# AlvinYH/Faster-VoxelPose

Hardware: AMD Instinct MI355X
Metric: frames/sec at 5-view 80x80x20 voxel (heatmaps -> 3D joints); MPJPE vs ref (mm) in mpjpe_vs_ref_mm (higher is better)
Workload: dtype f32

## Files before the change

faster-voxelpose_amd/csrc/fvp_project.hip:

```cpp
#include <hip/hip_runtime.h>

#include <cfloat>
#include <climits>
#include <cstdlib>

#include "fvp_common.h"
#include "fvp_geom.h"

namespace fvp {

template <int NV>
__global__ void __launch_bounds__(256) k_heat_to_cl(const float* __restrict__ heat, float* __restrict__ cl,
                                                    int J, int HW) {
  const int pix = blockIdx.x * 256 + threadIdx.x;
  const size_t bv = blockIdx.y;
  if (pix >= HW) return;
  const float* src = heat + bv * size_t(J) * HW + pix;
  float v[4 * NV];
#pragma unroll
  for (int j = 0; j < 4 * NV; ++j) v[j] = (j < J) ? src[size_t(j) * HW] : 0.0f;
  float4* dst = reinterpret_cast<float4*>(cl + (bv * HW + pix) * size_t(4 * NV));
#pragma unroll
  for (int q = 0; q < NV; ++q) dst[q] = make_float4(v[4 * q], v[4 * q + 1], v[4 * q + 2], v[4 * q + 3]);
}
// ... 1360 lines not shown
  if (B == 0) return 0;
  ProfScope ps(FVP_K_PROJECT_WHOLE, as_stream(s));
  const int threads = ceil_div(4 * Z, 64) * 64;
  if (g->JP <= 16)
    hipLaunchKernelGGL(k_project_columns_q<1>, dim3(B * N), dim3(threads), 0, as_stream(s), heat_cl,
                       reinterpret_cast<const Cam*>(cams), frame_set, ax, ay, az, Y, Z, X * Y, N, *g,
                       reinterpret_cast<const long long*>(flat), feat1d);
  else
    hipLaunchKernelGGL(k_project_columns_q<2>, dim3(B * N), dim3(threads), 0, as_stream(s), heat_cl,
                       reinterpret_cast<const Cam*>(cams), frame_set, ax, ay, az, Y, Z, X * Y, N, *g,
                       reinterpret_cast<const long long*>(flat), feat1d);
  return launch_status();
}

extern "C" int fvp_zmax(const float* cubes, float* zmax, long n, int Z, fvp_stream_t s) {
  FVP_REQUIRE(cubes && zmax && n >= 0 && Z > 0);
  if (n == 0) return 0;
  hipLaunchKernelGGL(k_zmax, dim3(unsigned((n + 255) / 256)), dim3(256), 0, as_stream(s), cubes, zmax, n, Z);
  return launch_status();
}

extern "C" int fvp_person_boxes(const float* centers, int n, const float* consts, const int32_t* fine_cube,
                                int32_t* boxes, float* offset, fvp_stream_t s) {
  FVP_REQUIRE(centers && consts && fine_cube && boxes && offset && n >= 0);
  if (n == 0) return 0;
  hipLaunchKernelGGL(k_person_boxes, dim3(ceil_div(n, 64)), dim3(64), 0, as_stream(s), centers, n, consts,
                     fine_cube[0], fine_cube[1], fine_cube[2], fine_cube[3], fine_cube[4], fine_cube[5], boxes,
                     offset);
  return launch_status();
}

extern "C" int fvp_plane_live_rows(const int32_t* boxes, int nP, int C, int32_t* live_rows, fvp_stream_t s) {
  FVP_REQUIRE(boxes && live_rows && nP >= 0 && C > 0);
  if (nP == 0) return 0;
  hipLaunchKernelGGL(k_plane_live_rows, dim3(ceil_div(nP, 64)), dim3(64), 0, as_stream(s), boxes, nP, C, live_rows);
  return launch_status();
}

static int check_cube(int C) {
  if (C < 4 || C > 256 || (C & (C - 1)) != 0) return FVP_ELIMIT;
  return 0;
}

extern "C" int fvp_project_individual(const float* heat_cl, const float* cams, const int32_t* frame_set,
                                      const int32_t* person_frame, const uint8_t* person_valid,
                                      const int32_t* boxes, const float* fx, const float* fy, const float* fz,
                                      const int32_t* fine, int C, int nP, const FvpGeom* g, float* cubes,
                                      fvp_stream_t s) {
  FVP_REQUIRE(heat_cl && cams && frame_set && person_frame && boxes && fx && fy && fz && cubes && nP >= 0);
  (void)fine;
  if (int e = check_geom(g)) return e;
  if (int e = check_cube(C)) return e;
  if (nP == 0) return 0;
  ProfScope ps(FVP_K_OTHER, as_stream(s));
#define CALL(NV)                                                                                                 \
  auto k = &k_project_individual<NV>;                                                                            \
  hipLaunchKernelGGL(k, dim3(ceil_div(C * C * C, 256), nP), dim3(256), 0, as_stream(s), heat_cl,                 \
                     reinterpret_cast<const Cam*>(cams), frame_set, person_frame, person_valid, boxes, fx, fy, fz, \
                     C, *g, cubes);
  FVP_NV_SWITCH(g->JP / 4, CALL)
#undef CALL
  return launch_status();
}

extern "C" int fvp_triplane_max(const float* cubes, float* planes, int nP, int J, int C, fvp_stream_t s) {
  FVP_REQUIRE(cubes && planes && nP >= 0 && J > 0);
  if (int e = check_cube(C)) return e;
  FVP_LIMIT(C <= 128);
  if (nP == 0) return 0;
  ProfScope ps(FVP_K_OTHER, as_stream(s));
  const int per = (C * C + 255) / 256;
  const dim3 grid(J, nP);
  const size_t lds = size_t(C) * (C + 1) * sizeof(float);
#define FVP_TRIMAX(PER_) hipLaunchKernelGGL(k_triplane_max<PER_>, grid, dim3(256), lds, as_stream(s), cubes, planes, J, C)
  if (per <= 1) FVP_TRIMAX(1);
  else if (per <= 4) FVP_TRIMAX(4);
  else if (per <= 16) FVP_TRIMAX(16);
  else FVP_TRIMAX(64);
#undef FVP_TRIMAX
  return launch_status();
}

static int tri_owned_ny(int C) { return ceil_div(C, kBY); }

extern "C" int fvp_project_individual_triplane(const float* heat_cl, const float* cams, const int32_t* frame_set,
                                               const int32_t* person_frame, const uint8_t* person_valid,
                                               const int32_t* boxes, const float* fx, const float* fy,
                                               const float* fz, const int32_t* fine, int C, int nP, const FvpGeom* g,
                                               float* planes, int persons_per_frame, const float* fine_grid,
                                               fvp_stream_t s) {
  FVP_REQUIRE(heat_cl && cams && frame_set && person_frame && boxes && fx && fy && fz && planes && nP >= 0);
  FVP_REQUIRE(!fine_grid || fine);
  if (int e = check_geom(g)) return e;
  if (int e = check_cube(C)) return e;
  if (nP == 0) return 0;
  const int ppf = (persons_per_frame > 0 && nP % persons_per_frame == 0) ? persons_per_frame : nP;
  [[maybe_unused]] const int chunks = ceil_div(C * C, 256);
  const int nvl = ceil_div(g->JP, 16);
  ProfScope ps(FVP_K_PROJECT_TRIPLANE, as_stream(s));
  const int F0 = fine_grid ? fine[0] : 0, F1 = fine_grid ? fine[1] : 0, F2 = fine_grid ? fine[2] : 0;
  const int nby = ceil_div(C, kBY);
#if FVP_DIAG
  const int nbx = ceil_div(C, kBX);
  static const bool gather = fvp::diag_env("FVP_TRIPLANE_GATHER") != nullptr;
  const bool quad_form = fvp::diag_env("FVP_TRIPLANE_QUAD") != nullptr;
  static const int tri_ablate_env = fvp::diag_env("FVP_TRI_ABLATE") ? atoi(fvp::diag_env("FVP_TRI_ABLATE")) : 0;
  const char* tt_env = fvp::diag_env("FVP_TRI_TWO_TILE");
  const bool staged = fvp::diag_env("FVP_TRIPLANE_STAGED") != nullptr;
  const bool force_lane = fvp::diag_env("FVP_TRIPLANE_LANE") != nullptr;
  const bool lane_form = !gather && !quad_form && g->JP <= 20 && ((staged && g->JP != 16) || force_lane);
  const int tri_ablate = (tri_ablate_env & ~16) | ((tt_env ? atoi(tt_env) != 0 : lane_form) ? 16 : 0);
  auto cap_lim = [](int cap) { const char* e = fvp::diag_env("FVP_TRI_CAP_PX"); const int v = e ? atoi(e) : cap; return v > 0 && v < cap ? v : cap; };
  const int cap_px = int((36 * 1024) / (size_t(g->JP) * 4));
  const size_t lds = 2 * size_t(cap_px) * g->JP * 4 + 64;
  if (lane_form) {
    const int lq = (g->JP / 4) | 1;
    const int cap_px = int((36 * 1024) / (size_t(lq) * 16));
    const size_t lds = 2 * size_t(cap_px) * lq * 16 + 64;
    FVP_LIMIT(size_t(cap_px) * lq * 4 >= size_t(kBX * kBY + (kBX + kBY) * 32) * g->JP);
#define CALL2(NQ_, CACHED_)                                                                                       \
  {                                                                                                                \
    static LdsOptIn optin;                                                                                         \
    auto k = &k_project_triplane_lds2<NQ_, CACHED_>;                                                              \
    if (int e = lds_opt_in(optin, reinterpret_cast<const void*>(k), lds)) return e;                                \
    hipLaunchKernelGGL(k, dim3(nbx * nby * nP), dim3(kTriThreads), lds, as_stream(s), heat_cl,                     \
                       reinterpret_cast<const Cam*>(cams), frame_set, person_frame, person_valid, boxes, fx, fy, fz, C, \
                       nP, nbx, nby, ppf, cap_px, *g, fine_grid, F0, F1, F2, planes, tri_ablate, cap_lim(cap_px));                  \
  }
#define CASE2(NQ_) case NQ_: if (fine_grid) CALL2(NQ_, true) else CALL2(NQ_, false) break;
    switch (g->JP / 4) {
      CASE2(1) CASE2(2) CASE2(3) CASE2(4) CASE2(5)
      default: return FVP_ELIMIT;
    }
#undef CASE2
#undef CALL2
    return launch_status();
  }
  const bool blk_form = !gather && !quad_form && !staged;
#else
  constexpr bool blk_form = true;
#endif
  if (blk_form && nvl <= 2) {
    const int nbx2 = ceil_div(C, kBlkBX);
    const int bz = nvl == 2 ? 16 : kBlkBZ;
    int zsh = 0;
    while ((1 << zsh) < C) ++zsh;
    const size_t lds_z = (size_t(kBlkBX + kBY) << zsh) * (g->JP + 1) * 4;
#if FVP_DIAG
    const char* zr_env = fvp::diag_env("FVP_TRI_ZRES");
    const bool zres = zr_env && atoi(zr_env) != 0 && (1 << zsh) >= bz && lds_z <= kTriZresMaxLds;
#else
    constexpr bool zres = false;
#endif
    const bool fits32 = (long long)g->H * g->W * g->JP * g->V <= INT_MAX && (long long)F0 * F1 * F2 * g->V <= INT_MAX;
    bool owned = tri_owned_lds(C, g->JP) <= kTriOwnMaxLds && fits32 && !zres;
    int ny = tri_owned_ny(C);
#if FVP_DIAG
    if (const char* e = fvp::diag_env("FVP_TRI_OWNED")) owned = owned && atoi(e) != 0;
    if (const char* e = fvp::diag_env("FVP_TRI_NY")) {
      const int v = atoi(e), top = ceil_div(C, kBY);
      ny = v < 1 ? 1 : (v > top ? top : v);
    }
#endif
    if (owned) {
      const int nsx = ceil_div(C, kOwnSX);
      int zsh_o = 0;
      while ((1 << zsh_o) < C || (1 << zsh_o) < kOwnBZ) ++zsh_o;
      const size_t lds_o = tri_owned_lds(C, g->JP);
      const bool q5o = nvl == 2 && g->JP == 20 && fvp::diag_env("FVP_TRI_NO_Q5") == nullptr;
#define CALLO(NVL_, CACHED_, Q5_)                                                                                            \
  hipLaunchKernelGGL((k_project_triplane_own<NVL_, CACHED_, Q5_>), dim3(nsx * ny * nP), dim3(kOwnThreads), lds_o,           \
                     as_stream(s), heat_cl, reinterpret_cast<const Cam*>(cams), frame_set, person_frame, person_valid, boxes, \
                     fx, fy, fz, C, nP, nsx, ny, ppf, *g, fine_grid, F0, F1, F2, planes, zsh_o)
      if (q5o) { if (fine_grid) CALLO(2, true, true); else CALLO(2, false, true); }
      else if (nvl == 2) { if (fine_grid) CALLO(2, true, false); else CALLO(2, false, false); }
      else { if (fine_grid) CALLO(1, true, false); else CALLO(1, false, false); }
#undef CALLO
      return launch_status();
    }
    const size_t lds_b = zres ? lds_z : size_t(kBlkBX * kBY + (kBlkBX + kBY) * bz) * (g->JP + 1) * 4;
#define CALLB(NVL_, CACHED_, ZRES_)                                                                                          \
  hipLaunchKernelGGL((k_project_triplane_blk<NVL_, CACHED_, ZRES_>), dim3(nbx2 * nby * nP), dim3(kBlkThreads), lds_b,       \
                     as_stream(s), heat_cl, reinterpret_cast<const Cam*>(cams), frame_set, person_frame, person_valid, boxes, \
                     fx, fy, fz, C, nP, nbx2, nby, ppf, *g, fine_grid, F0, F1, F2, planes, zsh)
#if FVP_DIAG
#define CALLB2(NVL_)                                                                     \
  {                                                                                      \
    if (fine_grid) { if (zres) CALLB(NVL_, true, true); else CALLB(NVL_, true, false); } \
    else { if (zres) CALLB(NVL_, false, true); else CALLB(NVL_, false, false); }         \
  }
#else
#define CALLB2(NVL_)                                                                     \
  {                                                                                      \
    if (fine_grid) CALLB(NVL_, true, false); else CALLB(NVL_, false, false);             \
  }
#endif
    const bool q5 = nvl == 2 && g->JP == 20 && !zres && fvp::diag_env("FVP_TRI_NO_Q5") == nullptr;
    if (q5) {
      if (fine_grid)
        hipLaunchKernelGGL((k_project_triplane_blk<2, true, false, true>), dim3(nbx2 * nby * nP), dim3(kBlkThreads), lds_b, as_stream(s),
                           heat_cl, reinterpret_cast<const Cam*>(cams), frame_set, person_frame, person_valid, boxes, fx, fy, fz, C, nP,
                           nbx2, nby, ppf, *g, fine_grid, F0, F1, F2, planes, zsh);
      else
        hipLaunchKernelGGL((k_project_triplane_blk<2, false, false, true>), dim3(nbx2 * nby * nP), dim3(kBlkThreads), lds_b, as_stream(s),
                           heat_cl, reinterpret_cast<const Cam*>(cams), frame_set, person_frame, person_valid, boxes, fx, fy, fz, C, nP,
                           nbx2, nby, ppf, *g, fine_grid, F0, F1, F2, planes, zsh);
    } else if (nvl == 2) CALLB2(2) else CALLB2(1)
#undef CALLB2
#undef CALLB
    return launch_status();
  }
#if FVP_DIAG
  if (!gather && nvl <= 2) {
    FVP_LIMIT(cap_px >= kBX * kBY + (kBX + kBY) * (nvl == 1 ? 32 : 16));
#define CALL(NVL_, CACHED_)                                                                                        \
  {                                                                                                                \
    static LdsOptIn optin;                                                                                         \
    auto k = &k_project_triplane_lds<NVL_, CACHED_>;                                                               \
    if (int e = lds_opt_in(optin, reinterpret_cast<const void*>(k), lds)) return e;                                \
    hipLaunchKernelGGL(k, dim3(nbx * nby * nP), dim3(kTriThreads), lds, as_stream(s), heat_cl,                     \
                       reinterpret_cast<const Cam*>(cams), frame_set, person_frame, person_valid, boxes, fx, fy, fz, C, \
                       nP, nbx, nby, ppf, cap_px, *g, fine_grid, F0, F1, F2, planes, tri_ablate, cap_lim(cap_px));                  \
  }
    if (nvl == 1) {
      if (fine_grid) CALL(1, true) else CALL(1, false)
    } else {
      if (fine_grid) CALL(2, true) else CALL(2, false)
    }
#undef CALL
    return launch_status();
  }
  if (nvl == 1) {
    auto k = &k_project_triplane<1>;
    hipLaunchKernelGGL(k, dim3(chunks * nP), dim3(1024), 0, as_stream(s), heat_cl, reinterpret_cast<const Cam*>(cams),
                       frame_set, person_frame, person_valid, boxes, fx, fy, fz, C, nP, chunks, ppf, *g, planes);
  } else if (nvl == 2) {
    auto k = &k_project_triplane<2>;
    hipLaunchKernelGGL(k, dim3(chunks * nP), dim3(1024), 0, as_stream(s), heat_cl, reinterpret_cast<const Cam*>(cams),
                       frame_set, person_frame, person_valid, boxes, fx, fy, fz, C, nP, chunks, ppf, *g, planes);
  } else {
    return FVP_ELIMIT;
  }
  return launch_status();
#else
  return FVP_ELIMIT;
#endif
}
```

faster-voxelpose_amd/csrc/fvp_project_lds.h:

```cpp
#pragma once
#include <type_traits>
#include <climits>

namespace fvp {

typedef float f32x2 __attribute__((ext_vector_type(2)));
#ifndef FVP_TRI_PACKED
#define FVP_TRI_PACKED 1
#endif
#ifndef FVP_TRI_EXPLICIT_AS
#define FVP_TRI_EXPLICIT_AS 1
#endif

typedef float f32x4v __attribute__((ext_vector_type(4)));
__device__ __forceinline__ float4 lds_ld4(const float* p) {
  const f32x4v v = *(const __attribute__((address_space(3))) f32x4v*)p;
  return make_float4(v.x, v.y, v.z, v.w);
}
__device__ __forceinline__ float4 glb_ld4(const float* p) {
  const f32x4v v = *(const __attribute__((address_space(1))) f32x4v*)p;
  return make_float4(v.x, v.y, v.z, v.w);
}

struct TapL {
// ... 552 lines not shown
    if (acc[0][0][0] != 1.2345e-30f) continue;
#endif
    if constexpr (ZRES) {
      int* rxz = reinterpret_cast<int*>(smem);
      int* ryz = rxz + ((kBX << zsh) * JPp);
      const int zb = gz0 - s2 + zs;
#pragma unroll
      for (int n = 0; n < NVL; ++n)
#pragma unroll
        for (int c = 0; c < 4; ++c) {
          const int ch = 16 * n + 4 * q + c;
          float mz = 0.0f;
#pragma unroll
          for (int i = 0; i < VPT; ++i) {
            const float val = fmaxf(acc[i][n][c], 0.0f);
            mz = fmaxf(mz, val);
            if (val > 0.0f && ch < JP) {
              const int z = zb + 4 * i;
              atomicMax(&rxz[((xx << zsh) + z) * JPp + ch], __float_as_int(val));
              atomicMax(&ryz[((yy << zsh) + z) * JPp + ch], __float_as_int(val));
            }
          }
          int mi = __float_as_int(mz);
          mi = imax(mi, dpp_i<0x124>(mi));
          mi = imax(mi, dpp_i<0x128>(mi));
          mxy[n][c] = imax(mxy[n][c], mi);
        }
      continue;
    }
    int* cxy = reinterpret_cast<int*>(smem);
    int* cxz = cxy + kBX * kBY * JPp;
    int* cyz = cxz + kBX * BZ * JPp;
    const int ncell = (kBX * kBY + (kBX + kBY) * BZ) * JPp;
    __syncthreads();
    for (int i = t; i < ncell; i += NT) cxy[i] = 0;
    __syncthreads();
#pragma unroll
    for (int n = 0; n < NVA; ++n)
#pragma unroll
      for (int c = 0; c < 4; ++c) {
        const int ch = 16 * n + 4 * q + c;
        float mz = 0.0f;
#pragma unroll
        for (int i = 0; i < VPT; ++i) {
          const float val = fmaxf(acc[i][n][c], 0.0f);
          mz = fmaxf(mz, val);
          if (val > 0.0f && ch < JP) {
            const int z = zs + 4 * i;
            atomicMax(&cxz[(xx * BZ + z) * JPp + ch], __float_as_int(val));
            atomicMax(&cyz[(yy * BZ + z) * JPp + ch], __float_as_int(val));
          }
        }
        int mi = __float_as_int(mz);
        mi = imax(mi, dpp_i<0x124>(mi));
        mi = imax(mi, dpp_i<0x128>(mi));
        if (zs == 0 && mi > 0 && ch < JP) cxy[(xx * kBY + yy) * JPp + ch] = mi;
      }
    if constexpr (Q5) {
#pragma unroll
      for (int c = 0; c < 4; ++c) {
        const int ch = 16 + c;
        float mz = 0.0f;
#pragma unroll
        for (int kk = 0; kk < OWN; ++kk) {
          const float val = fmaxf(accx[kk][0][c], 0.0f);
          mz = fmaxf(mz, val);
          if (val > 0.0f) {
            const int z = zs + 4 * (4 * kk + q);
            atomicMax(&cxz[(xx * BZ + z) * JPp + ch], __float_as_int(val));
            atomicMax(&cyz[(yy * BZ + z) * JPp + ch], __float_as_int(val));
          }
        }
        int mi = __float_as_int(mz);
        mi = imax(mi, dpp_i<0x121>(mi));
        mi = imax(mi, dpp_i<0x122>(mi));
        mi = imax(mi, dpp_i<0x124>(mi));
        mi = imax(mi, dpp_i<0x128>(mi));
        if (zs == 0 && q == 0 && mi > 0) cxy[(xx * kBY + yy) * JPp + ch] = mi;
      }
    }
    __syncthreads();
    const int lz0 = gz0 - tl2;
    for (int i = t; i < kBX * kBY * J; i += NT) {
      const int ch = i / (kBX * kBY), col = i - ch * (kBX * kBY), cx = col / kBY, cy = col - cx * kBY;
      const int raw = cxy[col * JPp + ch];
      if (raw > 0 && gx0 + cx < e0 && gy0 + cy < e1) {
        const int vv = __float_as_int(clampf(__fdiv_rn(__int_as_float(raw), nv), 0.0f, 1.0f));
        if (vv > 0) plane_max(&pxy[size_t(ch) * CC + (gx0 + cx - tl0) * C + (gy0 + cy - tl1)], vv);
      }
    }
    for (int i = t; i < (kBX + kBY) * BZ * J; i += NT) {
      const int ch = i / ((kBX + kBY) * BZ), r = i - ch * ((kBX + kBY) * BZ), a = r / BZ, z = r - a * BZ;
      if (gz0 + z < e2) {
        const int raw = cxz[r * JPp + ch];
        const int vv = raw > 0 ? __float_as_int(clampf(__fdiv_rn(__int_as_float(raw), nv), 0.0f, 1.0f)) : 0;
        if (vv > 0) {
          if (a < kBX) {
            if (gx0 + a < e0) plane_max(&pxz[size_t(ch) * CC + (gx0 + a - tl0) * C + lz0 + z], vv);
          } else if (gy0 + a - kBX < e1) {
            plane_max(&pyz[size_t(ch) * CC + (gy0 + a - kBX - tl1) * C + lz0 + z], vv);
          }
        }
      }
    }
  }
  if constexpr (ZRES) {
    __syncthreads();
    if (zs == 0 && col_in) {
#pragma unroll
      for (int n = 0; n < NVL; ++n)
#pragma unroll
        for (int c = 0; c < 4; ++c) {
          const int ch = 16 * n + 4 * q + c;
          if (ch < J && mxy[n][c] > 0) {
            const int vv = __float_as_int(clampf(__fdiv_rn(__int_as_float(mxy[n][c]), nv), 0.0f, 1.0f));
            if (vv > 0) plane_max(&pxy[size_t(ch) * CC + (gxi - tl0) * C + (gyi - tl1)], vv);
          }
        }
    }
    const int* cz = reinterpret_cast<const int*>(smem);
    const int nz = e2 - s2, lz0 = s2 - tl2;
    const int rows = (kBX + kBY) << zsh;
    for (int i = t; i < rows * J; i += NT) {
      static_assert(kBX + kBY == 8, "row count is a power of two");
      const int ch = i >> (zsh + 3), r = i & (rows - 1), a = r >> zsh, z = r & (zt - 1);
      if (z < nz) {
        const int raw = cz[r * JPp + ch];
        const int vv = raw > 0 ? __float_as_int(clampf(__fdiv_rn(__int_as_float(raw), nv), 0.0f, 1.0f)) : 0;
        if (vv > 0) {
          if (a < kBX) {
            if (gx0 + a < e0) plane_max(&pxz[size_t(ch) * CC + (gx0 + a - tl0) * C + lz0 + z], vv);
          } else if (gy0 + a - kBX < e1) {
            plane_max(&pyz[size_t(ch) * CC + (gy0 + a - kBX - tl1) * C + lz0 + z], vv);
          }
        }
      }
    }
  }
}

constexpr int kOwnSX = 4;
constexpr int kOwnBZ = 16;
constexpr int kOwnThreads = kOwnSX * kBY * 4 * 4;
#ifndef FVP_TRI_OWN_MAX_KB
#define FVP_TRI_OWN_MAX_KB 36
#endif
constexpr size_t kTriOwnMaxLds = size_t(FVP_TRI_OWN_MAX_KB) * 1024;
constexpr int kOwnPar = 16;
inline size_t tri_owned_lds(int C, int JP) {
  const int zt = C > kOwnBZ ? C : kOwnBZ;
  return (size_t(kOwnSX) * zt + 2 * size_t(kBY) * kOwnBZ) * size_t(JP + 1) * 4 + 4 * kOwnPar;
}

template <int NVL, bool CACHED, bool Q5 = false>
__global__ void __launch_bounds__(kOwnThreads, FVP_TRI_BLK_OCC)
k_project_triplane_own(const float* __restrict__ heat_cl, const Cam* __restrict__ cams, const int* __restrict__ frame_set,
                       const int* __restrict__ person_frame, const uint8_t* __restrict__ person_valid,
                       const int* __restrict__ boxes, const float* __restrict__ fx, const float* __restrict__ fy,
                       const float* __restrict__ fz, int C, int nP, int nsx, int ny, int ppf, FvpGeom g,
                       const float* __restrict__ fgrid, int F0, int F1, int F2, float* __restrict__ planes, int zsh) {
  static_assert(!Q5 || NVL == 2, "the five-quad form replaces the two-group form");
  constexpr int NVA = Q5 ? 1 : NVL;
  constexpr int BZ = kOwnBZ, VPT = BZ / 4, OWN = VPT / 4, SX = kOwnSX, NT = kOwnThreads;
  HIP_DYNAMIC_SHARED(float, smem)
  const int J = g.J, JP = g.JP, V = g.V, W = g.W, H = g.H;
  int p, blk;
  {
    const int id = blockIdx.x;
    const int bpp = nsx * ny, bpf = ppf * bpp;
    const int nframes = nP / ppf;
    if (nframes % 8 == 0) {
      const int xcd = id & 7, j = id >> 3;
      const int frame = xcd + 8 * (j / bpf), r = j % bpf;
      p = frame * ppf + r / bpp;
      blk = r % bpp;
    } else {
      p = id / bpp;
      blk = id % bpp;
    }
  }
  if (person_valid && !person_valid[p]) return;
  const int* bx = boxes + p * 9;
  const int tl0 = bx[0], tl1 = bx[1], tl2 = bx[2];
  const int zt = 1 << zsh;
  const int s0 = bx[3], s1 = bx[4], s2 = bx[5], e0 = bx[6], e1 = bx[7], e2 = imin(bx[8], s2 + zt);
  if (s0 >= e0 || s1 >= e1 || s2 >= e2) return;
  const int xs = blk / ny, seg = blk - xs * ny;
  const int gx0 = s0 + xs * SX;
  if (gx0 >= e0) return;
  const int nyb = (e1 - s1 + kBY - 1) / kBY, per = (nyb + ny - 1) / ny;
  if (seg * per >= nyb) return;
  const int ybeg = s1 + seg * per * kBY, yend = imin(ybeg + per * kBY, e1);

  const int t = threadIdx.x, q = t & 3;
  const int slot = t >> 2, zs = slot & 3, yy = (slot >> 2) & (kBY - 1), xx = slot / (4 * kBY);
  const int gxi = gx0 + xx;
  const bool x_in = gxi < e0;
  const int b = person_frame[p], set = frame_set[b];
  const int view_stride = H * W * JP;
  const float* frame = heat_cl + size_t(b) * V * view_stride;
  const Cam* cm = cams + size_t(set) * V;
  const float wx = x_in ? fx[gxi] : 0.0f;
  const int nfine = F0 * F1 * F2;
  const float2* gset = CACHED ? reinterpret_cast<const float2*>(fgrid) + size_t(set) * V * nfine : nullptr;
  const int JPp = JP + 1;
  int* rxz = reinterpret_cast<int*>(smem);
  int* ryz = rxz + ((SX << zsh) * JPp);
  constexpr int kYzCells = kBY * BZ;
  static_assert(kOwnPar >= 11, "merge-phase values");
  int* par = ryz + 2 * kYzCells * JPp;
  {
    const int ncell = ((SX << zsh) + 2 * kYzCells) * JPp;
    for (int i = t; i < ncell; i += NT) rxz[i] = 0;
    if (t == 0) {
      par[0] = p;
      par[1] = tl0 * C + tl1;
      par[2] = tl0 * C + tl2;
      par[3] = tl1 * C + tl2;
      par[4] = gx0;
      par[5] = e0;
      par[6] = s2;
      par[7] = yend;
      par[8] = C;
      par[9] = J;
      par[10] = ny;
    }
  }
  __syncthreads();
  auto parv = [&](int i) { return __builtin_amdgcn_readfirstlane(par[i]); };
  auto plane = [&](int person, int k) { return planes + (size_t(person) * 3 + k) * parv(9) * parv(8) * parv(8); };

  int kb = 0;
  for (int gy0 = ybeg; gy0 < parv(7); gy0 += kBY) {
    const int gyi = gy0 + yy;
    const bool col_in = x_in && gyi < parv(7);
    const float wy = col_in ? fy[gyi] : 0.0f;
    const unsigned colo = unsigned((col_in ? gxi : 0) * F1 + (col_in ? gyi : 0)) * unsigned(F2);
    float mcol[NVA][4];
#pragma unroll
    for (int n = 0; n < NVA; ++n)
#pragma unroll
      for (int c = 0; c < 4; ++c) mcol[n][c] = 0.0f;
    [[maybe_unused]] float mcol5[4] = {0.0f, 0.0f, 0.0f, 0.0f};

    for (int gz0 = parv(6); gz0 < e2; gz0 += BZ, ++kb) {
      float acc[VPT][NVA][4];
#pragma unroll
      for (int i = 0; i < VPT; ++i)
#pragma unroll
        for (int n = 0; n < NVA; ++n)
#pragma unroll
          for (int c = 0; c < 4; ++c) acc[i][n][c] = 0.0f;
      [[maybe_unused]] float accx[OWN][1][4];
#pragma unroll
      for (int kk = 0; kk < OWN; ++kk)
#pragma unroll
        for (int c = 0; c < 4; ++c) accx[kk][0][c] = 0.0f;
      float2 crd[OWN];
      auto load_coords = [&](int v) {
#pragma unroll
        for (int k = 0; k < OWN; ++k) {
          const int gzi = gz0 + zs + 4 * (q + 4 * k);
          crd[k] = (gset + size_t(v) * nfine)[colo + unsigned(gzi < F2 ? gzi : F2 - 1)];
        }
      };
      if (CACHED) load_coords(0);
      for (int v = 0; v < V; ++v) {
        TapL mine[OWN];
#pragma unroll
        for (int k = 0; k < OWN; ++k) {
          const int gzi = gz0 + zs + 4 * (q + 4 * k);
          const bool vin = col_in && gzi < e2;
          TapL d;
          d.base = kTapSkip;
          d.dx = d.dy = 0;
          d.w[0] = d.w[1] = d.w[2] = d.w[3] = 0.0f;
          if (vin) {
            float sx, sy;
            if (CACHED) {
              sx = crd[k].x;
              sy = crd[k].y;
            } else {
              project_norm(cm[v], g, wx, wy, fz[gzi], sx, sy);
            }
            int x0, y0, inside;
            float w4[4];
            tap_origin(sx, sy, W, H, x0, y0, w4, inside);
            const int cx0 = imin(imax(x0, 0), W - 1), cx1 = imin(imax(x0 + 1, 0), W - 1);
            const int cy0 = imin(imax(y0, 0), H - 1), cy1 = imin(imax(y0 + 1, 0), H - 1);
            d.base = ((cy0 * W + cx0) * JP) | tap_skip_mask(x0, y0, W, H);
            d.dx = (cx1 - cx0) * JP;
            d.dy = (cy1 - cy0) * W * JP;
#pragma unroll
            for (int c = 0; c < 4; ++c) d.w[c] = ((inside >> c) & 1) ? w4[c] : 0.0f;
          }
          mine[k] = d;
        }
        if (CACHED && v + 1 < V) load_coords(v + 1);
        const float* gsrc = frame + size_t(v) * view_stride;
        auto sample = [&](const TapL& tv, auto& a, auto own) {
          constexpr bool kOwn = decltype(own)::value;
#pragma unroll
          for (int n = 0; n < (kOwn ? 1 : NVA); ++n) {
            const int ch0 = kOwn ? 16 : 16 * n + 4 * q;
            if ((kOwn || n + 1 < NVL || ch0 < JP) && tap_contributes(tv)) {
              const float* p0 = gsrc + tv.base + ch0;
              const float4 v0 = glb_ld4(p0), v1 = glb_ld4(p0 + tv.dx), v2 = glb_ld4(p0 + tv.dy), v3 = glb_ld4(p0 + tv.dy + tv.dx);
              const f32x2 w0 = f32x2{tv.w[0], tv.w[0]}, w1 = f32x2{tv.w[1], tv.w[1]}, w2 = f32x2{tv.w[2], tv.w[2]},
                          w3 = f32x2{tv.w[3], tv.w[3]};
              f32x2 lo = f32x2{v0.x, v0.y} * w0, hi = f32x2{v0.z, v0.w} * w0;
              lo = __builtin_elementwise_fma(f32x2{v1.x, v1.y}, w1, lo);
              hi = __builtin_elementwise_fma(f32x2{v1.z, v1.w}, w1, hi);
              lo = __builtin_elementwise_fma(f32x2{v2.x, v2.y}, w2, lo);
              hi = __builtin_elementwise_fma(f32x2{v2.z, v2.w}, w2, hi);
              lo = __builtin_elementwise_fma(f32x2{v3.x, v3.y}, w3, lo);
              hi = __builtin_elementwise_fma(f32x2{v3.z, v3.w}, w3, hi);
              const f32x2 alo = f32x2{a[n][0], a[n][1]} + lo, ahi = f32x2{a[n][2], a[n][3]} + hi;
              a[n][0] = alo.x; a[n][1] = alo.y; a[n][2] = ahi.x; a[n][3] = ahi.y;
            }
          }
        };
#pragma unroll
        for (int k = 0; k < OWN; ++k) {
          { const TapL tv = quad_bcast_l<0>(mine[k]); sample(tv, acc[4 * k + 0], std::false_type{}); }
          { const TapL tv = quad_bcast_l<1>(mine[k]); sample(tv, acc[4 * k + 1], std::false_type{}); }
          { const TapL tv = quad_bcast_l<2>(mine[k]); sample(tv, acc[4 * k + 2], std::false_type{}); }
          { const TapL tv = quad_bcast_l<3>(mine[k]); sample(tv, acc[4 * k + 3], std::false_type{}); }
          if constexpr (Q5) sample(mine[k], accx[k], std::true_type{});
        }
      }
      int* cyz = ryz + (kb & 1) * (kYzCells * JPp);
      const int zb = gz0 - parv(6) + zs;
#pragma unroll
      for (int n = 0; n < NVA; ++n)
#pragma unroll
        for (int c = 0; c < 4; ++c) {
          const int ch = 16 * n + 4 * q + c;
#pragma unroll
          for (int i = 0; i < VPT; ++i) {
            const float val = fmaxf(acc[i][n][c], 0.0f);
            mcol[n][c] = fmaxf(mcol[n][c], val);
            if (val > 0.0f && ch < JP) {
              atomicMax(&rxz[((xx << zsh) + zb + 4 * i) * JPp + ch], __float_as_int(val));
              atomicMax(&cyz[(yy * BZ + zs + 4 * i) * JPp + ch], __float_as_int(val));
            }
          }
        }
      if constexpr (Q5) {
#pragma unroll
        for (int c = 0; c < 4; ++c) {
          const int ch = 16 + c;
#pragma unroll
          for (int kk = 0; kk < OWN; ++kk) {
            const float val = fmaxf(accx[kk][0][c], 0.0f);
            mcol5[c] = fmaxf(mcol5[c], val);
            if (val > 0.0f) {
              const int i = 4 * kk + q;
              atomicMax(&rxz[((xx << zsh) + zb + 4 * i) * JPp + ch], __float_as_int(val));
              atomicMax(&cyz[(yy * BZ + zs + 4 * i) * JPp + ch], __float_as_int(val));
            }
          }
        }
      }
      __syncthreads();
      float* pyz = plane(parv(0), 2) - parv(3);
      const float nv = float(V);
      const int Jm = parv(9), Cm = parv(8), CCm = Cm * Cm, yendm = parv(7);
      for (int i = t; i < kYzCells * Jm; i += NT) {
        static_assert(kYzCells == 64 && BZ == 16, "index arithmetic below");
        const int ch = i >> 6, r = i & 63, a = r >> 4, z = r & 15;
        const int raw = cyz[r * JPp + ch];
        if (raw > 0) {
          cyz[r * JPp + ch] = 0;
          if (gz0 + z < e2 && gy0 + a < yendm) {
            const int vv = __float_as_int(clampf(__fdiv_rn(__int_as_float(raw), nv), 0.0f, 1.0f));
            if (vv > 0) plane_max(&pyz[size_t(ch) * CCm + (gy0 + a) * Cm + gz0 + z], vv);
          }
        }
      }
    }
    const int Cx = parv(8), CCx = Cx * Cx;
    const int jl = (zs == 0 && col_in) ? parv(9) : 0;
    float* pxy = plane(parv(0), 0) - parv(1) + (gxi * Cx + gyi);
    const float nv = float(V);
#pragma unroll
    for (int n = 0; n < NVA; ++n)
#pragma unroll
      for (int c = 0; c < 4; ++c) {
        const int ch = 16 * n + 4 * q + c;
        int mi = __float_as_int(mcol[n][c]);
        mi = imax(mi, dpp_i<0x124>(mi));
        mi = imax(mi, dpp_i<0x128>(mi));
        if (ch < jl) pxy[size_t(ch) * CCx] = clampf(__fdiv_rn(__int_as_float(mi), nv), 0.0f, 1.0f);
      }
    if constexpr (Q5) {
#pragma unroll
      for (int c = 0; c < 4; ++c) {
        const int ch = 16 + c;
        int mi = __float_as_int(mcol5[c]);
        mi = imax(mi, dpp_i<0x121>(mi));
        mi = imax(mi, dpp_i<0x122>(mi));
        mi = imax(mi, dpp_i<0x124>(mi));
        mi = imax(mi, dpp_i<0x128>(mi));
        if (q == 0 && ch < jl) pxy[size_t(ch) * CCx] = clampf(__fdiv_rn(__int_as_float(mi), nv), 0.0f, 1.0f);
      }
    }
  }
  __syncthreads();
  {
    const int s2t = parv(6), nz = e2 - s2t, sgx0 = parv(4), se0 = parv(5), Jt = parv(9), Ct = parv(8), CCt = Ct * Ct, nyt = parv(10);
    float* pxz = plane(parv(0), 1) - parv(2) + s2t;
    const float nv = float(V);
    for (int i = t; i < (SX << zsh) * Jt; i += NT) {
      static_assert(SX == 4, "index arithmetic below");
      const int ch = i >> (zsh + 2), r = i & ((SX << zsh) - 1), a = r >> zsh, z = r & (zt - 1);
      if (z < nz && sgx0 + a < se0) {
        const int raw = rxz[r * JPp + ch];
        const int vv = raw > 0 ? __float_as_int(clampf(__fdiv_rn(__int_as_float(raw), nv), 0.0f, 1.0f)) : 0;
        float* cell = &pxz[size_t(ch) * CCt + (sgx0 + a) * Ct + z];
        if (nyt == 1) *cell = __int_as_float(vv);
        else if (vv > 0) plane_max(cell, vv);
      }
    }
  }
}

#if FVP_DIAG
template <int NQ, bool CACHED>
__global__ void __launch_bounds__(kTriThreads, 4)
k_project_triplane_lds2(const float* __restrict__ heat_cl, const Cam* __restrict__ cams, const int* __restrict__ frame_set,
                        const int* __restrict__ person_frame, const uint8_t* __restrict__ person_valid,
                        const int* __restrict__ boxes, const float* __restrict__ fx, const float* __restrict__ fy,
                        const float* __restrict__ fz, int C, int nP, int nbx, int nby, int ppf, int cap_px, FvpGeom g,
                        const float* __restrict__ fgrid, int F0, int F1, int F2, float* __restrict__ planes, int ablate, int cap_lim) {
  constexpr int BZ = 32, VPT = 2, JP = 4 * NQ;
  constexpr int LQ = NQ | 1, LP = 4 * LQ;
  HIP_DYNAMIC_SHARED(float, smem)
  constexpr int NT = kTriThreads;
  const int J = g.J, CC = C * C, V = g.V, W = g.W, H = g.H;
  const int tile_sz = cap_px * LP;
  int* rect = reinterpret_cast<int*>(smem + 2 * size_t(tile_sz));
  int p, blk;
  {
    const int id = blockIdx.x;
    const int bpp = nbx * nby, bpf = ppf * bpp;
    const int nframes = nP / ppf;
    if (nframes % 8 == 0) {
      const int xcd = id & 7, j = id >> 3;
      const int frame = xcd + 8 * (j / bpf), r = j % bpf;
      p = frame * ppf + r / bpp;
      blk = r % bpp;
    } else {
      p = id / bpp;
      blk = id % bpp;
    }
  }
  if (person_valid && !person_valid[p]) return;
  const int* bx = boxes + p * 9;
  const int tl0 = bx[0], tl1 = bx[1], tl2 = bx[2];
  const int s0 = bx[3], s1 = bx[4], s2 = bx[5], e0 = bx[6], e1 = bx[7], e2 = bx[8];
  if (s0 >= e0 || s1 >= e1 || s2 >= e2) return;
  const int xb = blk / nby, yb = blk - xb * nby;
  const int gx0 = s0 + xb * kBX, gy0 = s1 + yb * kBY;
  if (gx0 >= e0 || gy0 >= e1) return;

  const int t = threadIdx.x, lane = t & 63, wave = t >> 6;
  const int z16 = t & 15, yy = (t >> 4) & (kBY - 1), xx = t >> 6;
  const int gxi = gx0 + xx, gyi = gy0 + yy;
  const bool col_in = gxi < e0 && gyi < e1;
  const int b = person_frame[p];
  const size_t view_stride = size_t(H) * W * JP;
  const float* frame = heat_cl + size_t(b) * V * view_stride;
  const Cam* cm = cams + size_t(frame_set[b]) * V;
  const float wx = col_in ? fx[gxi] : 0.0f, wy = col_in ? fy[gyi] : 0.0f;
  const size_t nfine = size_t(F0) * F1 * F2;
  const float2* gcol = CACHED ? reinterpret_cast<const float2*>(fgrid) + size_t(frame_set[b]) * V * nfine +
                                    (size_t(col_in ? gxi : 0) * F1 + (col_in ? gyi : 0)) * F2
                              : nullptr;
  float* pxy = planes + (size_t(p) * 3 + 0) * J * CC;
  float* pxz = planes + (size_t(p) * 3 + 1) * J * CC;
  float* pyz = planes + (size_t(p) * 3 + 2) * J * CC;
  const float nv = float(V);

  struct Own { int xy[VPT]; int inside[VPT]; float w[VPT][4]; };
  float2 crd[VPT];
  auto load_coords = [&](int v, int gz0) {
#pragma unroll
    for (int k = 0; k < VPT; ++k) {
      const int gzi = gz0 + z16 + 16 * k;
      crd[k] = gcol[size_t(v) * nfine + (gzi < F2 ? gzi : F2 - 1)];
    }
  };
  auto project = [&](int v, int gz0, Own& o) {
    int mnx = INT_MIN, mxx = INT_MIN, mny = INT_MIN, mxy = INT_MIN;
#pragma unroll
    for (int k = 0; k < VPT; ++k) {
      const int gzi = gz0 + z16 + 16 * k;
      const bool vin = col_in && gzi < e2;
      o.inside[k] = 0;
      o.xy[k] = 0;
      o.w[k][0] = o.w[k][1] = o.w[k][2] = o.w[k][3] = 0.0f;
      if (vin) {
        float sx, sy;
        if (CACHED) {
          sx = crd[k].x;
          sy = crd[k].y;
        } else {
          project_norm(cm[v], g, wx, wy, fz[gzi], sx, sy);
        }
        int x0, y0;
        tap_origin(sx, sy, W, H, x0, y0, o.w[k], o.inside[k]);
        o.xy[k] = int((unsigned(y0) << 16) | (unsigned(x0) & 0xffffu));
// ... 189 lines not shown
```

Baseline: 3368.

## Use byte-offset tap records and cross-iteration coord prefetch in owned triplane kernel

For the single-group (NVA==1) path, tap records now carry four precomputed byte offsets in place of base/dx/dy, and are broadcast with raw DPP ops. This cuts per-sample address arithmetic and 64-bit pointer math. Cached grid coordinates are now prefetched across z-block boundaries, so the first view of the next block is already loaded. The occupancy hint for the NVL==1 cached variant is raised to 6, and LDS atomic addresses are precomputed per thread. Extra safety check on 32-bit byte offsets is added; ablation macros are included but off by default.

```diff
diff --git a/faster-voxelpose_amd/csrc/fvp_project.hip b/faster-voxelpose_amd/csrc/fvp_project.hip
--- a/faster-voxelpose_amd/csrc/fvp_project.hip
+++ b/faster-voxelpose_amd/csrc/fvp_project.hip
@@ -1536,7 +1536,8 @@
 #else
     constexpr bool zres = false;
 #endif
-    const bool fits32 = (long long)g->H * g->W * g->JP * g->V <= INT_MAX && (long long)F0 * F1 * F2 * g->V <= INT_MAX;
+    const bool fits32 = (long long)g->H * g->W * g->JP * g->V <= INT_MAX && (long long)F0 * F1 * F2 * g->V <= INT_MAX &&
+                        (long long)g->H * g->W * g->JP * 4 <= INT_MAX;
     bool owned = tri_owned_lds(C, g->JP) <= kTriOwnMaxLds && fits32 && !zres;
     int ny = tri_owned_ny(C);
 #if FVP_DIAG
diff --git a/faster-voxelpose_amd/csrc/fvp_project_lds.h b/faster-voxelpose_amd/csrc/fvp_project_lds.h
--- a/faster-voxelpose_amd/csrc/fvp_project_lds.h
+++ b/faster-voxelpose_amd/csrc/fvp_project_lds.h
@@ -728,8 +728,23 @@
   return (size_t(kOwnSX) * zt + 2 * size_t(kBY) * kOwnBZ) * size_t(JP + 1) * 4 + 4 * kOwnPar;
 }
 
+struct TapO { int o[4]; float w[4]; };
+constexpr int kTapSkipO = INT_MIN;
+template <int SRC>
+__device__ __forceinline__ int quad_bcast_b(int v) { return __builtin_amdgcn_update_dpp(0, v, SRC * 0x55, 0xf, 0xf, true); }
+__device__ __forceinline__ float4 glb_ld4b(const char* base, unsigned off) {
+  const f32x4v v = *(const __attribute__((address_space(1))) f32x4v*)(base + off);
+  return make_float4(v.x, v.y, v.z, v.w);
+}
+#ifndef FVP_TRI_OWN_OCC1
+#define FVP_TRI_OWN_OCC1 6
+#endif
+#ifndef FVP_TRI_ABLATE
+#define FVP_TRI_ABLATE 0
+#endif
+
 template <int NVL, bool CACHED, bool Q5 = false>
-__global__ void __launch_bounds__(kOwnThreads, FVP_TRI_BLK_OCC)
+__global__ void __launch_bounds__(kOwnThreads, (NVL == 1 && CACHED) ? FVP_TRI_OWN_OCC1 : FVP_TRI_BLK_OCC)
 k_project_triplane_own(const float* __restrict__ heat_cl, const Cam* __restrict__ cams, const int* __restrict__ frame_set,
                        const int* __restrict__ person_frame, const uint8_t* __restrict__ person_valid,
                        const int* __restrict__ boxes, const float* __restrict__ fx, const float* __restrict__ fy,
@@ -780,6 +795,7 @@
   const int nfine = F0 * F1 * F2;
   const float2* gset = CACHED ? reinterpret_cast<const float2*>(fgrid) + size_t(set) * V * nfine : nullptr;
   const int JPp = JP + 1;
+  const int JP4 = JP * 4, q16 = 16 * q;
   int* rxz = reinterpret_cast<int*>(smem);
   int* ryz = rxz + ((SX << zsh) * JPp);
   constexpr int kYzCells = kBY * BZ;
@@ -819,6 +835,19 @@
       for (int c = 0; c < 4; ++c) mcol[n][c] = 0.0f;
     [[maybe_unused]] float mcol5[4] = {0.0f, 0.0f, 0.0f, 0.0f};
 
+    [[maybe_unused]] float2 crd[OWN];
+    auto load_step = [&](int n, int gz) {
+      if (n >= V) { n = 0; gz += BZ; }
+      if (gz < e2) {
+#pragma unroll
+        for (int k = 0; k < OWN; ++k) {
+          const int gzi = gz + zs + 4 * (q + 4 * k);
+          crd[k] = (gset + size_t(n) * nfine)[colo + unsigned(gzi < F2 ? gzi : F2 - 1)];
+        }
+      }
+    };
+    if (CACHED && !(FVP_TRI_ABLATE & 4)) load_step(0, parv(6));
+
     for (int gz0 = parv(6); gz0 < e2; gz0 += BZ, ++kb) {
       float acc[VPT][NVA][4];
 #pragma unroll
@@ -832,81 +861,183 @@
       for (int kk = 0; kk < OWN; ++kk)
 #pragma unroll
         for (int c = 0; c < 4; ++c) accx[kk][0][c] = 0.0f;
-      float2 crd[OWN];
-      auto load_coords = [&](int v) {
-#pragma unroll
-        for (int k = 0; k < OWN; ++k) {
-          const int gzi = gz0 + zs + 4 * (q + 4 * k);
-          crd[k] = (gset + size_t(v) * nfine)[colo + unsigned(gzi < F2 ? gzi : F2 - 1)];
-        }
-      };
-      if (CACHED) load_coords(0);
       for (int v = 0; v < V; ++v) {
-        TapL mine[OWN];
-#pragma unroll
-        for (int k = 0; k < OWN; ++k) {
-          const int gzi = gz0 + zs + 4 * (q + 4 * k);
-          const bool vin = col_in && gzi < e2;
-          TapL d;
-          d.base = kTapSkip;
-          d.dx = d.dy = 0;
-          d.w[0] = d.w[1] = d.w[2] = d.w[3] = 0.0f;
-          if (vin) {
-            float sx, sy;
-            if (CACHED) {
-              sx = crd[k].x;
-              sy = crd[k].y;
-            } else {
-              project_norm(cm[v], g, wx, wy, fz[gzi], sx, sy);
+        if constexpr (NVA == 1) {
+          TapO mine[OWN];
+#pragma unroll
+          for (int k = 0; k < OWN; ++k) {
+            const int gzi = gz0 + zs + 4 * (q + 4 * k);
+            const bool vin = col_in && gzi < e2;
+            TapO d;
+            d.o[0] = kTapSkipO;
+            d.o[1] = d.o[2] = d.o[3] = 0;
+            d.w[0] = d.w[1] = d.w[2] = d.w[3] = 0.0f;
+#if FVP_TRI_ABLATE & 4
+            if (vin) {
+              d.o[0] = (((gzi & 15) + 3 * v) * W + 2 * (gyi & 7) + (gxi & 3)) * JP4;
+              d.o[1] = d.o[0] + JP4, d.o[2] = d.o[0] + W * JP4, d.o[3] = d.o[2] + JP4;
+              d.w[0] = 0.4f, d.w[1] = 0.3f, d.w[2] = 0.2f, d.w[3] = 0.1f;
             }
-            int x0, y0, inside;
-            float w4[4];
-            tap_origin(sx, sy, W, H, x0, y0, w4, inside);
-            const int cx0 = imin(imax(x0, 0), W - 1), cx1 = imin(imax(x0 + 1, 0), W - 1);
-            const int cy0 = imin(imax(y0, 0), H - 1), cy1 = imin(imax(y0 + 1, 0), H - 1);
-            d.base = ((cy0 * W + cx0) * JP) | tap_skip_mask(x0, y0, W, H);
-            d.dx = (cx1 - cx0) * JP;
-            d.dy = (cy1 - cy0) * W * JP;
-#pragma unroll
-            for (int c = 0; c < 4; ++c) d.w[c] = ((inside >> c) & 1) ? w4[c] : 0.0f;
-          }
-          mine[k] = d;
-        }
-        if (CACHED && v + 1 < V) load_coords(v + 1);
-        const float* gsrc = frame + size_t(v) * view_stride;
-        auto sample = [&](const TapL& tv, auto& a, auto own) {
-          constexpr bool kOwn = decltype(own)::value;
-#pragma unroll
-          for (int n = 0; n < (kOwn ? 1 : NVA); ++n) {
-            const int ch0 = kOwn ? 16 : 16 * n + 4 * q;
-            if ((kOwn || n + 1 < NVL || ch0 < JP) && tap_contributes(tv)) {
-              const float* p0 = gsrc + tv.base + ch0;
-              const float4 v0 = glb_ld4(p0), v1 = glb_ld4(p0 + tv.dx), v2 = glb_ld4(p0 + tv.dy), v3 = glb_ld4(p0 + tv.dy + tv.dx);
-              const f32x2 w0 = f32x2{tv.w[0], tv.w[0]}, w1 = f32x2{tv.w[1], tv.w[1]}, w2 = f32x2{tv.w[2], tv.w[2]},
-                          w3 = f32x2{tv.w[3], tv.w[3]};
-              f32x2 lo = f32x2{v0.x, v0.y} * w0, hi = f32x2{v0.z, v0.w} * w0;
-              lo = __builtin_elementwise_fma(f32x2{v1.x, v1.y}, w1, lo);
-              hi = __builtin_elementwise_fma(f32x2{v1.z, v1.w}, w1, hi);
-              lo = __builtin_elementwise_fma(f32x2{v2.x, v2.y}, w2, lo);
-              hi = __builtin_elementwise_fma(f32x2{v2.z, v2.w}, w2, hi);
-              lo = __builtin_elementwise_fma(f32x2{v3.x, v3.y}, w3, lo);
-              hi = __builtin_elementwise_fma(f32x2{v3.z, v3.w}, w3, hi);
-              const f32x2 alo = f32x2{a[n][0], a[n][1]} + lo, ahi = f32x2{a[n][2], a[n][3]} + hi;
-              a[n][0] = alo.x; a[n][1] = alo.y; a[n][2] = ahi.x; a[n][3] = ahi.y;
+            if (false) {
+#else
+            if (vin) {
+#endif
+              float sx, sy;
+              if (CACHED) {
+                sx = crd[k].x;
+                sy = crd[k].y;
+              } else {
+                project_norm(cm[v], g, wx, wy, fz[gzi], sx, sy);
+              }
+              int x0, y0, inside;
+              float w4[4];
+              tap_origin(sx, sy, W, H, x0, y0, w4, inside);
+              const int cx0 = imin(imax(x0, 0), W - 1), cx1 = imin(imax(x0 + 1, 0), W - 1);
+              const int cy0 = imin(imax(y0, 0), H - 1), cy1 = imin(imax(y0 + 1, 0), H - 1);
+              const int dxb = (cx1 - cx0) * JP4, dyb = (cy1 - cy0) * W * JP4;
+              d.o[0] = ((cy0 * W + cx0) * JP4) | (tap_skip_mask(x0, y0, W, H) & kTapSkipO);
+              d.o[1] = d.o[0] + dxb;
+              d.o[2] = d.o[0] + dyb;
+              d.o[3] = d.o[2] + dxb;
+#pragma unroll
+              for (int c = 0; c < 4; ++c) d.w[c] = ((inside >> c) & 1) ? w4[c] : 0.0f;
             }
-          }
-        };
-#pragma unroll
-        for (int k = 0; k < OWN; ++k) {
-          { const TapL tv = quad_bcast_l<0>(mine[k]); sample(tv, acc[4 * k + 0], std::false_type{}); }
-          { const TapL tv = quad_bcast_l<1>(mine[k]); sample(tv, acc[4 * k + 1], std::false_type{}); }
-          { const TapL tv = quad_bcast_l<2>(mine[k]); sample(tv, acc[4 * k + 2], std::false_type{}); }
-          { const TapL tv = quad_bcast_l<3>(mine[k]); sample(tv, acc[4 * k + 3], std::false_type{}); }
-          if constexpr (Q5) sample(mine[k], accx[k], std::true_type{});
-        }
-      }
+            mine[k] = d;
+          }
+          if (CACHED && !(FVP_TRI_ABLATE & 4)) load_step(v + 1, gz0);
+          const char* gsrc = reinterpret_cast<const char*>(frame + size_t(v) * view_stride);
+          struct Pass { int u[4]; float w[4]; };
+          auto bcast = [&](const TapO& m, auto src) {
+            constexpr int SRC = decltype(src)::value;
+            Pass ps;
+#pragma unroll
+            for (int j = 0; j < 4; ++j) ps.u[j] = quad_bcast_b<SRC>(m.o[j]) + q16;
+#pragma unroll
+            for (int j = 0; j < 4; ++j) ps.w[j] = __int_as_float(quad_bcast_b<SRC>(__float_as_int(m.w[j])));
+            return ps;
+          };
+          auto loads = [&](const Pass& ps, float4 (&r)[4]) {
+#pragma unroll
+            for (int j = 0; j < 4; ++j) {
+#if FVP_TRI_ABLATE & 1
+              r[j] = make_float4(ps.w[j], ps.w[3 - j], float(ps.u[j]), 1.0f);
+#else
+              r[j] = glb_ld4b(gsrc, unsigned(ps.u[j]));
+#endif
+            }
+          };
+          auto fmas = [&](const Pass& ps, const float4 (&r)[4], float (&a)[4]) {
+            const f32x2 w0 = f32x2{ps.w[0], ps.w[0]}, w1 = f32x2{ps.w[1], ps.w[1]}, w2 = f32x2{ps.w[2], ps.w[2]},
+                        w3 = f32x2{ps.w[3], ps.w[3]};
+            f32x2 lo = f32x2{r[0].x, r[0].y} * w0, hi = f32x2{r[0].z, r[0].w} * w0;
+            lo = __builtin_elementwise_fma(f32x2{r[1].x, r[1].y}, w1, lo);
+            hi = __builtin_elementwise_fma(f32x2{r[1].z, r[1].w}, w1, hi);
+            lo = __builtin_elementwise_fma(f32x2{r[2].x, r[2].y}, w2, lo);
+            hi = __builtin_elementwise_fma(f32x2{r[2].z, r[2].w}, w2, hi);
+            lo = __builtin_elementwise_fma(f32x2{r[3].x, r[3].y}, w3, lo);
+            hi = __builtin_elementwise_fma(f32x2{r[3].z, r[3].w}, w3, hi);
+            const f32x2 alo = f32x2{a[0], a[1]} + lo, ahi = f32x2{a[2], a[3]} + hi;
+            a[0] = alo.x; a[1] = alo.y; a[2] = ahi.x; a[3] = ahi.y;
+          };
+          const bool quad_in = NVL > 1 || 4 * q < JP;
+          auto pass = [&](const Pass& ps, float (&a)[4]) {
+            if (ps.u[0] >= 0 && quad_in) {
+              float4 r[4];
+              loads(ps, r);
+              fmas(ps, r, a);
+            }
+          };
+#pragma unroll
+          for (int k = 0; k < OWN; ++k) {
+            pass(bcast(mine[k], std::integral_constant<int, 0>{}), acc[4 * k + 0][0]);
+            pass(bcast(mine[k], std::integral_constant<int, 1>{}), acc[4 * k + 1][0]);
+            pass(bcast(mine[k], std::integral_constant<int, 2>{}), acc[4 * k + 2][0]);
+            pass(bcast(mine[k], std::integral_constant<int, 3>{}), acc[4 * k + 3][0]);
+            if constexpr (Q5) {
+              Pass p5;
+#pragma unroll
+              for (int j = 0; j < 4; ++j) { p5.u[j] = mine[k].o[j] + 64; p5.w[j] = mine[k].w[j]; }
+              if (p5.u[0] >= 0) {
+                float4 r[4];
+                loads(p5, r);
+                fmas(p5, r, accx[k][0]);
+              }
+            }
+          }
+        } else {
+          TapL mine[OWN];
+#pragma unroll
+          for (int k = 0; k < OWN; ++k) {
+            const int gzi = gz0 + zs + 4 * (q + 4 * k);
+            const bool vin = col_in && gzi < e2;
+            TapL d;
+            d.base = kTapSkip;
+            d.dx = d.dy = 0;
+            d.w[0] = d.w[1] = d.w[2] = d.w[3] = 0.0f;
+            if (vin) {
+              float sx, sy;
+              if (CACHED) {
+                sx = crd[k].x;
+                sy = crd[k].y;
+              } else {
+                project_norm(cm[v], g, wx, wy, fz[gzi], sx, sy);
+              }
+              int x0, y0, inside;
+              float w4[4];
+              tap_origin(sx, sy, W, H, x0, y0, w4, inside);
+              const int cx0 = imin(imax(x0, 0), W - 1), cx1 = imin(imax(x0 + 1, 0), W - 1);
+              const int cy0 = imin(imax(y0, 0), H - 1), cy1 = imin(imax(y0 + 1, 0), H - 1);
+              d.base = ((cy0 * W + cx0) * JP) | tap_skip_mask(x0, y0, W, H);
+              d.dx = (cx1 - cx0) * JP;
+              d.dy = (cy1 - cy0) * W * JP;
+#pragma unroll
+              for (int c = 0; c < 4; ++c) d.w[c] = ((inside >> c) & 1) ? w4[c] : 0.0f;
+            }
+            mine[k] = d;
+          }
+          if (CACHED) load_step(v + 1, gz0);
+          const float* gsrc = frame + size_t(v) * view_stride;
+          auto sample = [&](const TapL& tv, auto& a, auto own) {
+            constexpr bool kOwn = decltype(own)::value;
+#pragma unroll
+            for (int n = 0; n < (kOwn ? 1 : NVA); ++n) {
+              const int ch0 = kOwn ? 16 : 16 * n + 4 * q;
+              if ((kOwn || n + 1 < NVL || ch0 < JP) && tap_contributes(tv)) {
+                const float* p0 = gsrc + tv.base + ch0;
+                const float4 v0 = glb_ld4(p0), v1 = glb_ld4(p0 + tv.dx), v2 = glb_ld4(p0 + tv.dy), v3 = glb_ld4(p0 + tv.dy + tv.dx);
+                const f32x2 w0 = f32x2{tv.w[0], tv.w[0]}, w1 = f32x2{tv.w[1], tv.w[1]}, w2 = f32x2{tv.w[2], tv.w[2]},
+                            w3 = f32x2{tv.w[3], tv.w[3]};
+                f32x2 lo = f32x2{v0.x, v0.y} * w0, hi = f32x2{v0.z, v0.w} * w0;
+                lo = __builtin_elementwise_fma(f32x2{v1.x, v1.y}, w1, lo);
+                hi = __builtin_elementwise_fma(f32x2{v1.z, v1.w}, w1, hi);
+                lo = __builtin_elementwise_fma(f32x2{v2.x, v2.y}, w2, lo);
+                hi = __builtin_elementwise_fma(f32x2{v2.z, v2.w}, w2, hi);
+                lo = __builtin_elementwise_fma(f32x2{v3.x, v3.y}, w3, lo);
+                hi = __builtin_elementwise_fma(f32x2{v3.z, v3.w}, w3, hi);
+                const f32x2 alo = f32x2{a[n][0], a[n][1]} + lo, ahi = f32x2{a[n][2], a[n][3]} + hi;
+                a[n][0] = alo.x; a[n][1] = alo.y; a[n][2] = ahi.x; a[n][3] = ahi.y;
+              }
+            }
+          };
+#pragma unroll
+          for (int k = 0; k < OWN; ++k) {
+            { const TapL tv = quad_bcast_l<0>(mine[k]); sample(tv, acc[4 * k + 0], std::false_type{}); }
+            { const TapL tv = quad_bcast_l<1>(mine[k]); sample(tv, acc[4 * k + 1], std::false_type{}); }
+            { const TapL tv = quad_bcast_l<2>(mine[k]); sample(tv, acc[4 * k + 2], std::false_type{}); }
+            { const TapL tv = quad_bcast_l<3>(mine[k]); sample(tv, acc[4 * k + 3], std::false_type{}); }
+            if constexpr (Q5) sample(mine[k], accx[k], std::true_type{});
+          }
+        }
+      }
+#if FVP_TRI_ABLATE & 2
+      if (acc[0][0][0] != 1.2345e-30f) { mcol[0][0] = fmaxf(mcol[0][0], acc[0][0][0] + acc[VPT - 1][NVA - 1][3] + (Q5 ? accx[0][0][0] : 0.0f)); continue; }
+#endif
       int* cyz = ryz + (kb & 1) * (kYzCells * JPp);
       const int zb = gz0 - parv(6) + zs;
+      [[maybe_unused]] int* lxz = rxz + (((xx << zsh) + zb) * JPp + 4 * q);
+      [[maybe_unused]] int* lyz = cyz + ((yy * BZ + zs) * JPp + 4 * q);
+      auto cell_xz = [&](int i, int w) { return CACHED ? lxz + i * (4 * JPp) + w : &rxz[((xx << zsh) + zb + 4 * i) * JPp + 4 * q + w]; };
+      auto cell_yz = [&](int i, int w) { return CACHED ? lyz + i * (4 * JPp) + w : &cyz[(yy * BZ + zs + 4 * i) * JPp + 4 * q + w]; };
 #pragma unroll
       for (int n = 0; n < NVA; ++n)
 #pragma unroll
@@ -917,23 +1048,22 @@
             const float val = fmaxf(acc[i][n][c], 0.0f);
             mcol[n][c] = fmaxf(mcol[n][c], val);
             if (val > 0.0f && ch < JP) {
-              atomicMax(&rxz[((xx << zsh) + zb + 4 * i) * JPp + ch], __float_as_int(val));
-              atomicMax(&cyz[(yy * BZ + zs + 4 * i) * JPp + ch], __float_as_int(val));
+              atomicMax(cell_xz(i, 16 * n + c), __float_as_int(val));
+              atomicMax(cell_yz(i, 16 * n + c), __float_as_int(val));
             }
           }
         }
       if constexpr (Q5) {
 #pragma unroll
         for (int c = 0; c < 4; ++c) {
-          const int ch = 16 + c;
 #pragma unroll
           for (int kk = 0; kk < OWN; ++kk) {
             const float val = fmaxf(accx[kk][0][c], 0.0f);
             mcol5[c] = fmaxf(mcol5[c], val);
             if (val > 0.0f) {
               const int i = 4 * kk + q;
-              atomicMax(&rxz[((xx << zsh) + zb + 4 * i) * JPp + ch], __float_as_int(val));
-              atomicMax(&cyz[(yy * BZ + zs + 4 * i) * JPp + ch], __float_as_int(val));
+              atomicMax(cell_xz(i, 16 + c - 4 * q), __float_as_int(val));
+              atomicMax(cell_yz(i, 16 + c - 4 * q), __float_as_int(val));
             }
           }
         }
```

Result: faster. 3406, median of 5 (+1.1%).
